# jinseokbae/neural_marionette

Measured on AMD Instinct MI355X. Metric: voxel-frames/sec (64^3, T=16), higher is better.
Workload: dtype f32 (conv products as 3x f16-split MFMA with f32 accumulate, fp32-equivalent; everything else f32); 1 GPU; AIST++-shaped synthetic clips 64^3 T=16 B=4/GPU, full NeuralMarionette.forward (detector + 11 losses + HSVRNNBVH.encode, best-of-10), fp32, random-init weights; grid=64, T=16, clips_per_gpu=4, global_clips=4, conv_mode=split16, parallelism=clip-sharded x1 (no data-path collective)

## Files before the change

### neural_marionette_amd/csrc/nm_conv.hip

```cpp
#include "nm_common.h"
#include "nm_up2c.h"
#include <type_traits>
#include <utility>
#include <vector>

namespace {

#define NM_SPLIT_SCALE 2048.0f

struct ConvParams {
    const float* in; const float* in_scale; const float* in_shift; float in_slope;
    int N, ID, IH, IW, Cin;
    const float* w; const float* bias;
    float* out; float* part;
    int OD, OH, OW, Cout, Co_pad;
    int ks, stride, pad;
    int bz_l2, by_l2, bx_l2;
    int nbz, nby, nbx;
    int KC;
    int cin_real;
    int up2;
    int HZ, HY, HX, HV, HVp;
    int CVp;
    int ZP;
    const void* w16;
    int ksplit;
    int st_z, st_y, st_x;
    unsigned st_sx, st_sy, st_pf;
    unsigned st_m_sx, st_m_sy, st_m_pf;
    const float* in_alt; const unsigned char* in_map;
    const float* in2; const float* in2_scale; const float* in2_shift; float in2_slope;
    int in_h, out_h;
#ifdef NM_DIAG
    unsigned long long* stamps;
#endif
};

__device__ __forceinline__ void lds_barrier() { asm volatile("s_waitcnt lgkmcnt(0)\n\ts_barrier" ::: "memory"); }

__device__ __forceinline__ float lrelu(float v, float slope) { return v > 0.f ? v : v * slope; }


template <bool IH = false>
__device__ __forceinline__ f32x4 load_raw(const ConvParams& p, int n, int z, int y, int x, int c) {
    return nm_ld4<IH>(p.in, ((((size_t)n * p.ID + z) * p.IH + y) * p.IW + x) * p.Cin + c);
}

__device__ __forceinline__ f32x4 apply_act(const ConvParams& p, f32x4 v, const f32x4& sc, const f32x4& sh) {
    if (p.in_scale) {
#pragma unroll
        for (int j = 0; j < 4; ++j) v[j] = __builtin_fmaf(v[j], sc[j], sh[j]);
    }
    if (p.in_slope != 1.0f) {
#pragma unroll
        for (int j = 0; j < 4; ++j) v[j] = fmaxf(v[j], v[j] * p.in_slope);
    }
    return v;
}

__device__ __forceinline__ f32x4 sum_act2(const ConvParams& p, f32x4 a, const f32x4& sca, const f32x4& sha, f32x4 b, const f32x4& scb, const f32x4& shb) {
#pragma unroll
    for (int j = 0; j < 4; ++j) {
        float u = a[j], v = b[j];
        if (p.in_scale) { u = u * sca[j]; u = u + sha[j]; }
        if (p.in_slope != 1.0f) u = u > 0.f ? u : u * p.in_slope;
        if (p.in2_scale) { v = v * scb[j]; v = v + shb[j]; }
        if (p.in2_slope != 1.0f) v = v > 0.f ? v : v * p.in2_slope;
        a[j] = u + v;
    }
    return a;
}

template <bool IH = false>
__device__ __forceinline__ f32x4 load_act(const ConvParams& p, int n, int z, int y, int x, int c) {
    f32x4 v = nm_ld4<IH>(p.in, ((((size_t)n * p.ID + z) * p.IH + y) * p.IW + x) * p.Cin + c);
    f32x4 sc = {0.f, 0.f, 0.f, 0.f}, sh = sc;
    if (p.in_scale) {
        sc = *reinterpret_cast<const f32x4*>(p.in_scale + (size_t)n * p.Cin + c);
        sh = *reinterpret_cast<const f32x4*>(p.in_shift + (size_t)n * p.Cin + c);
    }
    return apply_act(p, v, sc, sh);
}

// ... 2105 lines not shown
            NM_MFMA2(accl[0][0], bh0[i], al0[i]);  if constexpr (bnext) bh0[j] = lds_read16_untracked<BN>(vb);
            NM_MFMA2(accl[0][1], bh1[i], al0[i]);  if constexpr (bnext) bh1[j] = lds_read16_untracked<BN + 32 * 16>(vb);
            NM_MFMA2(acc[1][0], bh0[i], ah1[i]);  if constexpr (bnext) bl0[j] = lds_read16_untracked<BN + 128 * 16>(vb);
            NM_MFMA2(acc[1][1], bh1[i], ah1[i]);  if constexpr (bnext) bl1[j] = lds_read16_untracked<BN + 160 * 16>(vb);
            NM_MFMA2(accl[1][0], bl0[i], ah1[i]);
            NM_MFMA2(accl[1][1], bl1[i], ah1[i]);
            NM_MFMA2(accl[1][0], bh0[i], al1[i]);
            NM_MFMA2(accl[1][1], bh1[i], al1[i]);
            if constexpr (t == 8) {
                NM_PSTAMP(1 + 2 * g);
                asm volatile("s_barrier" ::: "memory");
                __builtin_amdgcn_sched_barrier(0);
                NM_PSTAMP(2 + 2 * g);
            }
        });
        gpar ^= 1;
        if (has_next) {
            ah0[0] = lds_read16_untracked<0>(van); al0[0] = lds_read16_untracked<LO>(van);
            ah1[0] = lds_read16_untracked<YO>(van); al1[0] = lds_read16_untracked<LO + YO>(van);
        }
        if (cur.cb == C16 - 1) {
            const Work& w = cur.w;
            NM_PSTAMP(8);
#pragma unroll
            for (int nt = 0; nt < 2; ++nt) {
                float s1[16], s2[16];
#pragma unroll
                for (int mt = 0; mt < 2; ++mt) {
                    const size_t dst = ((((size_t)w.n * p.OD + w.oz0 + vz) * p.OH + w.oy0 + 2 * wave + mt) * p.OW + w.ox0 + vx) * (size_t)p.Cout +
                                       w.cg * 64 + nt * 32 + 4 * h;
#pragma unroll
                    for (int k4 = 0; k4 < 4; ++k4) {
                        const f32x4 b4 = *reinterpret_cast<const f32x4*>(lbias + w.cg * 64 + nt * 32 + 8 * k4 + 4 * h);
                        f32x4 v;
#pragma unroll
                        for (int e = 0; e < 4; e += 2) {
                            const f32x2 a2 = f32x2{acc[mt][nt][4 * k4 + e], acc[mt][nt][4 * k4 + e + 1]};
                            const f32x2 l2 = f32x2{accl[mt][nt][4 * k4 + e], accl[mt][nt][4 * k4 + e + 1]};
                            const f32x2 v2 = (a2 + l2 * (1.0f / NM_SPLIT_SCALE)) + f32x2{b4[e], b4[e + 1]};
                            const f32x2 q2 = v2 * v2;
                            v[e] = v2[0]; v[e + 1] = v2[1];
                            if (mt == 0) { s1[4 * k4 + e] = v2[0]; s1[4 * k4 + e + 1] = v2[1]; s2[4 * k4 + e] = q2[0]; s2[4 * k4 + e + 1] = q2[1]; }
                            else {
                                const f32x2 t1 = f32x2{s1[4 * k4 + e], s1[4 * k4 + e + 1]} + v2, t2 = f32x2{s2[4 * k4 + e], s2[4 * k4 + e + 1]} + q2;
                                s1[4 * k4 + e] = t1[0]; s1[4 * k4 + e + 1] = t1[1]; s2[4 * k4 + e] = t2[0]; s2[4 * k4 + e + 1] = t2[1];
                            }
                            acc[mt][nt][4 * k4 + e] = 0.f; acc[mt][nt][4 * k4 + e + 1] = 0.f; accl[mt][nt][4 * k4 + e] = 0.f; accl[mt][nt][4 * k4 + e + 1] = 0.f;
                        }
                        *reinterpret_cast<f32x4*>(p.out + dst + 8 * k4) = v;
                    }
                }
                if (nt == 0) NM_PSTAMP(9); else NM_PSTAMP(11);
                if (p.part) {
                    dpp_sum32_many(s1); dpp_sum32_many(s2);
                    if (l31 == 16) {
#pragma unroll
                        for (int r = 0; r < 16; ++r)
                            *reinterpret_cast<f32x2*>(red + (wave * 64 + nt * 32 + (r & 3) + 8 * (r >> 2) + 4 * h) * 2) = f32x2{s1[r], s2[r]};
                    }
                }
                if (nt == 0) NM_PSTAMP(10);
            }
            NM_PSTAMP(12);
            lds_barrier();
            NM_PSTAMP(13);
            if (p.part && tid < 64) {
                float a = 0.f, b = 0.f;
#pragma unroll
                for (int q = 0; q < 4; ++q) { a += red[(q * 64 + tid) * 2]; b += red[(q * 64 + tid) * 2 + 1]; }
                const int br = ((w.oz0 >> 2) * nby + (w.oy0 >> 3)) * nbx + (w.ox0 >> 3);
                float* dp = p.part + (((size_t)w.n * nbr + br) * p.Cout + w.cg * 64 + tid) * 2;
                dp[0] = a; dp[1] = b;
            }
        }
        NM_PSTAMP(7);
#ifdef NM_DIAG
        ++step_no;
#endif
        if (!has_next) break;
        cur = nxt; hb ^= 1;
    }
}

template <int IO = 0>
__global__ __launch_bounds__(512, 1) void conv_f16q2_kernel(ConvParams p) {
    constexpr bool IH = (IO & 1) != 0, OH = (IO & 2) != 0;
    constexpr unsigned EB = IH ? 2u : 4u;
    constexpr int HV = 600, ZP = 100, HX = 10;
    constexpr int WB = 27 * 2 * 64;
    constexpr int NP = IH ? 5 : 10;
    constexpr int NCH = IH ? 8 : 4;
    constexpr int NWL = 14;
    constexpr int NA = IH ? 4 : 2;
    extern __shared__ f32x4 lds[];
    half8* ldh = reinterpret_cast<half8*>(lds);
    half8* ldb = ldh + 4 * HV;
    float* red = reinterpret_cast<float*>(ldb + 2 * WB);
    float* lbias = red + 512;
    const int tid = threadIdx.x, lane = tid & 63, wave = __builtin_amdgcn_readfirstlane(tid >> 6);
    const int h = lane >> 5, l31 = lane & 31;
    const int C16 = p.Cin >> 4;
    const int ncg = p.Cout >> 6;
    const int nbx = p.OW >> 3, nby = p.OH >> 3, nbz = p.OD >> 2, nbr = nbx * nby * nbz;
    const int total = p.N * nbr * ncg;
    const int per = (total + (int)gridDim.x - 1) / (int)gridDim.x;
    const int id_first = (int)blockIdx.x * per, id_last = min(total, id_first + per);
    if (id_first >= id_last) return;

    struct Work { int n, oz0, oy0, ox0, cg; };
    const bool tiled = p.st_x != 0;
    auto decode = [&](int id) {
        Work w;
        if (tiled) {
            const BrickPos bp = super_tile_item(p, (int)blockIdx.x, id - id_first, per, nbz, nby, nbx);
            w.cg = 0; w.n = bp.n; w.ox0 = bp.bx << 3; w.oy0 = bp.by << 3; w.oz0 = bp.bz << 2;
            return w;
        }
        w.cg = id % ncg; const int bid = id / ncg;
        w.n = bid / nbr; const int br = bid % nbr;
        w.ox0 = (br % nbx) << 3; w.oy0 = ((br / nbx) % nby) << 3; w.oz0 = (br / (nbx * nby)) << 2;
        return w;
    };
    auto next_work = [&](Work w, int id) {
        if (tiled) return decode(id);
        if (++w.cg == ncg) {
            w.cg = 0;
            if ((w.ox0 += 8) == p.OW) { w.ox0 = 0; if ((w.oy0 += 8) == p.OH) { w.oy0 = 0; if ((w.oz0 += 4) == p.OD) { w.oz0 = 0; ++w.n; } } }
        }
        return w;
    };
    struct Step { Work w; int id, cb; };
    auto advance = [&](Step& st) {
        if (st.cb + 1 < C16) { ++st.cb; return true; }
        if (st.id + 1 >= id_last) return false;
        st.cb = 0; ++st.id; st.w = next_work(st.w, st.id);
        return true;
    };

    if (wave >= 4) {
        const int pt = tid - 256, pw = wave - 4;
        const half8* __restrict__ w8 = reinterpret_cast<const half8*>(p.w);
        const size_t plane = (size_t)p.Co_pad;
        const int sub = IH ? (pt & 1) : (pt & 3);
        int pc_slot[NP], pc_rel[NP], pc_pos[NP];
#pragma unroll
        for (int k = 0; k < NP; ++k) {
            const int v = IH ? (pt >> 1) + 128 * k : (pt >> 2) + 64 * k, vc = min(v, HV - 1);
            const int hz = vc / 100, r = vc % 100, hy = r / 10, hx = r % 10;
            pc_slot[k] = (IH ? sub : (sub >> 1)) * HV + hz * ZP + hy * HX + hx;
            pc_rel[k] = ((hz * p.IH + hy) * p.IW + hx) * p.Cin + NCH * sub;
            pc_pos[k] = (v < HV) ? (hz | (hy << 8) | (hx << 16)) : -1;
        }
        f32x4 raw[2][NP], sc[2][NA / 2], sh[2][NA / 2], wreg[NWL];
#pragma unroll
        for (int i = 0; i < NWL; ++i) wreg[i] = f32x4{0.f, 0.f, 0.f, 0.f};
        const bool has_affine = p.in_scale != nullptr;
        const unsigned rel111 = (unsigned)(((p.IH + 1) * p.IW + 1) * p.Cin) * EB;
        auto inside_mask = [&](const Work& w) {
            unsigned m = 0;
#pragma unroll
            for (int k = 0; k < NP; ++k) {
                const int hz = pc_pos[k] & 0xff, hy = (pc_pos[k] >> 8) & 0xff, hx = pc_pos[k] >> 16;
                const bool in = pc_pos[k] >= 0 && (unsigned)(w.oz0 - 1 + hz) < (unsigned)p.ID && (unsigned)(w.oy0 - 1 + hy) < (unsigned)p.IH &&
                                (unsigned)(w.ox0 - 1 + hx) < (unsigned)p.IW;
                m |= (in ? 1u : 0u) << k;
            }
// ... 588 lines not shown
    return e;
}

double conv_flops(const ConvParams& p, double taps) { return 2.0 * p.N * (double)p.OD * p.OH * p.OW * p.Cout * (double)p.cin_real * taps; }

template <int MT, int NT>
int launch_t(const ConvParams& p, const Tiling& t, dim3 grid, hipStream_t s) {
    static NmDeviceOnce attr_set;
    if (int rc = nm_raise_lds_limit(attr_set, 160 * 1024, "hipFuncSetAttribute(conv)", &conv_mfma_kernel<MT, NT>)) return rc;
    NmProfScope prof(s, conv_flops(p, (double)p.ks * p.ks * p.ks), (MT - 1) * 2 + (NT - 1));
    hipLaunchKernelGGL((conv_mfma_kernel<MT, NT>), grid, dim3(256), t.lds_bytes, s, p);
    return nm_check_hip(hipGetLastError(), "conv_mfma launch");
}

void choose_super_tile(ConvParams& p, int nblocks, int nbz, int nby, int nbx) {
    p.st_z = p.st_y = p.st_x = 0;
    p.st_sx = p.st_sy = p.st_pf = p.st_m_sx = p.st_m_sy = p.st_m_pf = 0;
    if (nblocks % 8) return;
    const int gs = nblocks / 8;
    const int sz = gs == 64 ? 4 : gs == 32 ? 2 : 0;
    if (!sz || nbz % sz || nby % 4 || nbx % 4) return;
    const long long st = (long long)p.N * (nbz / sz) * (nby / 4) * (nbx / 4);
    if (st % 8 || st / 8 * nblocks != (long long)p.N * nbz * nby * nbx) return;
    p.st_z = sz; p.st_y = 4; p.st_x = 4;
    const unsigned SX = (unsigned)nbx / 4u, SY = (unsigned)nby / 4u, pf = SX * SY * (unsigned)(nbz / sz);
    const unsigned long long smax = 8ull * (unsigned long long)(((long long)p.N * nbz * nby * nbx + nblocks - 1) / nblocks) + 8ull;
    auto magic = [](unsigned d) { return d == 1u ? 0u : (unsigned)((0x100000000ull + d - 1ull) / d); };
    if (smax * pf < 0x100000000ull) {
        p.st_sx = SX; p.st_sy = SY; p.st_pf = pf; p.st_m_sx = magic(SX); p.st_m_sy = magic(SY); p.st_m_pf = magic(pf);
    }
}


template <int MT, int NT, int KS, bool UP2, bool SINGLE, int IO = 0>
int launch_f16s_impl(const ConvParams& p_in, const Tiling& t, dim3 grid, hipStream_t s) {
    ConvParams p = p_in;
    static NmDeviceOnce attr_set;
    if (int rc = nm_raise_lds_limit(attr_set, 160 * 1024, "hipFuncSetAttribute(conv_f16s)", &conv_f16s_kernel<MT, NT, KS, UP2, SINGLE, IO>)) return rc;
    dim3 pgrid(min(grid.x, 512u), grid.y);
    choose_super_tile(p, (int)pgrid.x, p.nbz, p.nby, p.nbx);
    NmProfScope prof(s, conv_flops(p, (double)p.ks * p.ks * p.ks), UP2 ? 10 + (NT - 1) : 5 + (NT - 1));
    hipLaunchKernelGGL((conv_f16s_kernel<MT, NT, KS, UP2, SINGLE, IO>), pgrid, dim3(256), t.lds_bytes, s, p);
    return nm_check_hip(hipGetLastError(), "conv_f16s launch");
}
int io16_unsupported(const char* k, const ConvParams& p) {
    nm_set_error("%s: no instantiation for bfloat16 input=%d / output=%d in this conv mode / layer shape (16-bit storage needs conv mode 4)", k, p.in_h, p.out_h);
    return NM_ERR_UNSUPPORTED;
}
template <int MT, int NT, int KS, bool UP2>
int launch_f16s(const ConvParams& p, const Tiling& t, dim3 grid, hipStream_t s) {
    const int io = (p.in_h ? 1 : 0) | (p.out_h ? 2 : 0);
    if (io) {
        if (!nm_ls().single) return io16_unsupported("conv_f16s", p);
        if constexpr (KS == 1 && !UP2) { if (io == 3) return launch_f16s_impl<MT, NT, KS, UP2, true, 3>(p, t, grid, s); }
        if constexpr (KS == 3 && UP2 && NT == 2) { if (io == 2) return launch_f16s_impl<MT, NT, KS, UP2, true, 2>(p, t, grid, s); }
        return io16_unsupported("conv_f16s", p);
    }
    return nm_ls().single ? launch_f16s_impl<MT, NT, KS, UP2, true>(p, t, grid, s) : launch_f16s_impl<MT, NT, KS, UP2, false>(p, t, grid, s);
}

template <int NT, bool SINGLE>
int launch_pool_f16s_impl(const ConvParams& p, dim3 grid, hipStream_t s) {
    const int io = (p.in_h ? 1 : 0) | (p.out_h ? 2 : 0);
    if (io && (!SINGLE || p.Cin > 128 || p.in2 || p.in_map || !(io & 1))) return io16_unsupported("conv_pool_f16q", p);
    NmProfScope prof(s, conv_flops(p, 8.0), 8);
    if (io) {
        if constexpr (SINGLE) {
            if (io == 3) hipLaunchKernelGGL((conv_pool_f16q_kernel<NT, true, false, 3>), grid, dim3(256), 0, s, p);
            else hipLaunchKernelGGL((conv_pool_f16q_kernel<NT, true, false, 1>), grid, dim3(256), 0, s, p);
        }
    } else
    if (nm_ls().pool_q && p.Cin <= 128) {
        if (p.in2) hipLaunchKernelGGL((conv_pool_f16q_kernel<NT, SINGLE, true>), grid, dim3(256), 0, s, p);
        else hipLaunchKernelGGL((conv_pool_f16q_kernel<NT, SINGLE, false>), grid, dim3(256), 0, s, p);
    } else
    hipLaunchKernelGGL((conv_pool_f16s_kernel<NT, SINGLE>), grid, dim3(256), 0, s, p);
    return nm_check_hip(hipGetLastError(), "conv_pool_f16s launch");
}
template <int NT>
int launch_pool_f16s(const ConvParams& p, dim3 grid, hipStream_t s) {
    return nm_ls().single ? launch_pool_f16s_impl<NT, true>(p, grid, s) : launch_pool_f16s_impl<NT, false>(p, grid, s);
}

template <auto KERNEL>
int launch_persistent(const char* what_attr, const char* what_launch, int variant, bool super_tile, const ConvParams& p_in,
                      size_t lds_bytes, int work_items, hipStream_t s, int wgs_cap) {
    static NmDeviceOnce attr_set;
    if (int rc = nm_raise_lds_limit(attr_set, 160 * 1024, what_attr, KERNEL)) return rc;
    const int cus = nm_num_cus();
    if (!cus) return NM_ERR_HIP;
    ConvParams p = p_in;
    const int wgs = wgs_cap > 0 && wgs_cap < cus ? min(cus, max(8, wgs_cap & ~7)) : cus;
    dim3 grid((unsigned)min(work_items, wgs));
    if (super_tile) choose_super_tile(p, (int)grid.x, p.OD / 4, p.OH / 8, p.OW / 8);
    NmProfScope prof(s, conv_flops(p, 27.0), variant);
    hipLaunchKernelGGL(KERNEL, grid, dim3(512), lds_bytes, s, p);
    return nm_check_hip(hipGetLastError(), what_launch);
}

template <bool SINGLE, int IO = 0>
int launch_f16p_impl(const ConvParams& p, int work_items, hipStream_t s, int wgs_cap) {
    const size_t lds_bytes = (size_t)8 * 600 * 16 + (size_t)3 * 9 * 4 * 32 * 16 + (size_t)(256 + p.Cout) * sizeof(float);
    return launch_persistent<&conv_f16p_kernel<SINGLE, IO>>("hipFuncSetAttribute(conv_f16p)", "conv_f16p launch", 7, p.Cout == 32, p, lds_bytes, work_items, s, wgs_cap);
}
int launch_f16p(const ConvParams& p, int work_items, hipStream_t s, int wgs_cap) {
    const int io = (p.in_h ? 1 : 0) | (p.out_h ? 2 : 0);
    if (io) {
        if (io != 3 || !nm_ls().single) return io16_unsupported("conv_f16p", p);
        return launch_f16p_impl<true, 3>(p, work_items, s, wgs_cap);
    }
    return nm_ls().single ? launch_f16p_impl<true>(p, work_items, s, wgs_cap) : launch_f16p_impl<false>(p, work_items, s, wgs_cap);
}

int launch_f16p2_impl(const ConvParams& p, int work_items, hipStream_t s, int wgs_cap) {
    const size_t lds_bytes = (size_t)8 * 600 * 16 + (size_t)2 * 9 * 4 * 64 * 16 + (size_t)(512 + p.Cout) * sizeof(float);
    return launch_persistent<&conv_f16p2_kernel>("hipFuncSetAttribute(conv_f16p2)", "conv_f16p2 launch", 9, p.Cout == 64, p, lds_bytes, work_items, s, wgs_cap);
}
template <int IO>
int launch_f16q2_impl(const ConvParams& p, int work_items, hipStream_t s, int wgs_cap) {
    const size_t lds_bytes = (size_t)4 * 600 * 16 + (size_t)2 * 27 * 2 * 64 * 16 + (size_t)(512 + p.Cout) * sizeof(float);
    if (lds_bytes > 160 * 1024) { nm_set_error("conv_f16q2: %d output channels exceed the LDS budget", p.Cout); return NM_ERR_UNSUPPORTED; }
    return launch_persistent<&conv_f16q2_kernel<IO>>("hipFuncSetAttribute(conv_f16q2)", "conv_f16q2 launch", 14, p.Cout == 64, p, lds_bytes, work_items, s, wgs_cap);
}
template <int IO, int C16T>
int launch_f16r_impl(const ConvParams& p, int work_items, hipStream_t s, int wgs_cap) {
    const size_t lds_bytes = (size_t)4 * 600 * 16 + (size_t)27 * C16T * 64 * 16 + (size_t)(512 + 32) * sizeof(float) + 2048 + 256 + 1024;
    return launch_persistent<&conv_f16r_kernel<IO, C16T>>("hipFuncSetAttribute(conv_f16r)", "conv_f16r launch", 15, true, p, lds_bytes, work_items, s, wgs_cap);
}
int launch_f16p2(const ConvParams& p, int work_items, hipStream_t s, int wgs_cap) {
    const int io = (p.in_h ? 1 : 0) | (p.out_h ? 2 : 0);
    if (io && (io != 3 || !nm_ls().single)) return io16_unsupported("conv_f16p2", p);
    if (nm_ls().single) return io ? launch_f16q2_impl<3>(p, work_items, s, wgs_cap) : launch_f16q2_impl<0>(p, work_items, s, wgs_cap);
    return launch_f16p2_impl(p, work_items, s, wgs_cap);
}

#ifdef NM_DIAG
unsigned long long* g_stamps = nullptr;
#endif

}

#ifdef NM_DIAG
extern "C" void nm_diag_set_stamps(void* p) { g_stamps = static_cast<unsigned long long*>(p); }
#endif
void nm_conv_set_mode(int mode) { NmLaunchState& l = nm_ls(); l.conv_mode = mode ? 1 : 0; l.f16p_all = mode == 2; l.single = mode == 3 || mode == 4; l.store16 = mode == 4; }
int nm_conv_get_mode() { const NmLaunchState& l = nm_ls(); return l.conv_mode && l.single ? (l.store16 ? 4 : 3) : (l.conv_mode && l.f16p_all ? 2 : l.conv_mode); }
int nm_conv_single() { return nm_ls().conv_mode && nm_ls().single; }

int nm_launch_pack_conv_weight16(const float* w, int Cout, int Cin, int ks, void* packed, int Co_pad, hipStream_t s) {
    if (Co_pad % 32 || Cout > Co_pad) { nm_set_error("pack_conv_weight16: bad padding Cout=%d/%d", Cout, Co_pad); return NM_ERR_ARG; }
    size_t total = (size_t)ks * ks * ks * ((Cin + 15) / 16) * 2 * Co_pad * 8;
    int blocks = (int)min((total + 255) / 256, (size_t)2048);
    hipLaunchKernelGGL(pack_conv_weight16_kernel, dim3(blocks), dim3(256), 0, s, w, Cout, Cin, ks, reinterpret_cast<_Float16*>(packed), Co_pad);
    return nm_check_hip(hipGetLastError(), "pack_conv_weight16 launch");
}

__global__ __launch_bounds__(256) void pack_jobs_kernel(const NmPackJob* __restrict__ jobs, int njobs) {
    int lo = 0, hi = njobs - 1;
    while (lo < hi) { const int mid = (lo + hi + 1) >> 1; if (jobs[mid].blk0 <= (int)blockIdx.x) lo = mid; else hi = mid - 1; }
    const NmPackJob j = jobs[lo];
    const int lb = blockIdx.x - j.blk0, taps = j.ks * j.ks * j.ks;
    auto W = [&](int co, int ci, int tap) -> float {
        if (co >= j.Cout || ci >= j.Cin) return 0.f;
        if (j.src_rows > 0 && ((j.flip ? ci : co) >= j.src_rows || (j.flip ? co : ci) >= j.src_cin)) return 0.f;
        return j.flip ? j.src[((size_t)ci * j.src_cin + co) * taps + (taps - 1 - tap)] : j.src[((size_t)co * j.src_cin + ci) * taps + tap];
    };
    const size_t total32 = (size_t)taps * j.Cin_pad * j.Co_pad;
    for (size_t i = (size_t)lb * 256 + threadIdx.x; i < total32; i += (size_t)j.nblk * 256) {
        const int e = i & 3; size_t r = i >> 2;
        const int co = r % j.Co_pad; r /= j.Co_pad;
        const int q = r % (j.Cin_pad / 4), tap = r / (j.Cin_pad / 4);
        j.wp[i] = W(co, q * 4 + e, tap);
    }
    if (j.wp16) {
        _Float16* packed = reinterpret_cast<_Float16*>(j.wp16);
        const int C16 = (j.Cin + 15) >> 4;
        const size_t total16 = (size_t)taps * C16 * 2 * j.Co_pad * 8;
        for (size_t i = (size_t)lb * 256 + threadIdx.x; i < total16; i += (size_t)j.nblk * 256) {
            const int e = i & 7; size_t r = i >> 3;
            const int co = r % j.Co_pad; r /= j.Co_pad;
            const int hh = r & 1; r >>= 1;
            const int cb = r % C16, tap = r / C16;
            const float v = W(co, cb * 16 + hh * 8 + e, tap);
            const _Float16 h = (_Float16)v;
            const _Float16 l = (_Float16)((v - (float)h) * NM_SPLIT_SCALE);
            const size_t base = ((((size_t)tap * C16 + cb) * 4) * j.Co_pad) * 8;
            packed[base + ((size_t)hh * j.Co_pad + co) * 8 + e] = h;
            packed[base + ((size_t)(2 + hh) * j.Co_pad + co) * 8 + e] = l;
        }
    }
}

int nm_pack_job_blocks(const NmPackJob& j) {
    const size_t total = (size_t)j.ks * j.ks * j.ks * j.Cin_pad * j.Co_pad;
// ... 83 lines not shown

void nm_conv_prof_reset() {
    NmLaunchState& l = nm_ls();
    for (const NmProfRec& r : l.prof) { l.event_pool.push_back(r.a); l.event_pool.push_back(r.b); }
    l.prof.clear();
}

int nm_launch_conv(const TensorRef& in, const float* w_packed, const float* bias, float* out,
                   const ConvGeom& g, float* part, hipStream_t s, int cin_real, const void* w_packed16, int out_h, int wgs_cap) {
    if (in.C % 8 != 0 || g.Co_pad % 32 != 0 || g.Cout > g.Co_pad || g.Cout <= 0) {
        nm_set_error("conv: unsupported channels Cin=%d Cout=%d Co_pad=%d", in.C, g.Cout, g.Co_pad);
        return NM_ERR_ARG;
    }
    const int us = g.up2 ? 2 : 1;
    if ((us * in.D + 2 * g.pad - g.ks) / g.stride + 1 != g.OD || (us * in.H + 2 * g.pad - g.ks) / g.stride + 1 != g.OH ||
        (us * in.W + 2 * g.pad - g.ks) / g.stride + 1 != g.OW) {
        nm_set_error("conv: geometry mismatch in=(%d,%d,%d) k=%d s=%d p=%d out=(%d,%d,%d)", in.D, in.H, in.W,
                     g.ks, g.stride, g.pad, g.OD, g.OH, g.OW);
        return NM_ERR_ARG;
    }
    if ((in.scale == nullptr) != (in.shift == nullptr)) { nm_set_error("conv: scale/shift must come together"); return NM_ERR_ARG; }
    if ((in.brickmap || in.p2) && g.up2) { nm_set_error("conv: a brick-sparse input tensor can only feed the k2 s2 split-fp16 pool kernel"); return NM_ERR_ARG; }
    if (use_up2c(g, in.C)) {
        double flops = 2.0 * in.N * (double)g.OD * g.OH * g.OW * g.Cout * (double)(cin_real > 0 ? cin_real : in.C) * 27.0;
        if (nm_up2y_active()) flops *= 0.5;
        NmProfScope prof(s, flops, 12);
        return nm_launch_conv_up2c(in, g.up2c, bias, out, g.Cout, g.Co_pad, part, s, out_h);
    }
    Tiling t = choose_tiling(g, in.C);
    if (t.lds_bytes > 160 * 1024) { nm_set_error("conv: LDS tile %zu B too large", t.lds_bytes); return NM_ERR_UNSUPPORTED; }
    ConvParams p;
    p.in = in.p; p.in_scale = in.scale; p.in_shift = in.shift; p.in_slope = in.slope;
    p.N = in.N; p.ID = in.D; p.IH = in.H; p.IW = in.W; p.Cin = in.C;
    p.w = w_packed; p.bias = bias; p.out = out; p.part = part;
    p.OD = g.OD; p.OH = g.OH; p.OW = g.OW; p.Cout = g.Cout; p.Co_pad = g.Co_pad;
    p.ks = g.ks; p.stride = g.stride; p.pad = g.pad;
    p.bz_l2 = t.bz_l2; p.by_l2 = t.by_l2; p.bx_l2 = t.bx_l2; p.nbz = t.nbz; p.nby = t.nby; p.nbx = t.nbx;
    p.cin_real = cin_real > 0 ? cin_real : in.C;
    p.up2 = g.up2 ? 1 : 0;
    p.st_z = p.st_y = p.st_x = 0;
    p.st_sx = p.st_sy = p.st_pf = p.st_m_sx = p.st_m_sy = p.st_m_pf = 0;
    p.in_alt = in.alt; p.in_map = in.brickmap;
    p.in2 = in.p2; p.in2_scale = in.scale2; p.in2_shift = in.shift2; p.in2_slope = in.slope2;
    p.in_h = in.h; p.out_h = out_h;
    if (in.p2 && !(nm_conv_pool16_eligible(in.C, g.OD, g.OH, g.OW, w_packed16 != nullptr) && g.ks == 2 && g.stride == 2 && g.pad == 0 && !g.up2 && !in.brickmap)) {
        nm_set_error("conv: an un-materialised residual sum can only feed the k2 s2 split-fp16 pool kernel"); return NM_ERR_ARG;
    }
    if (in.brickmap && !(nm_conv_pool16_eligible(in.C, g.OD, g.OH, g.OW, w_packed16 != nullptr) && g.ks == 2 && g.stride == 2 && g.pad == 0 && !g.up2 &&
                         in.alt && in.D % 4 == 0 && in.H % 8 == 0 && in.W % 8 == 0)) {
        nm_set_error("conv: a brick-sparse input tensor can only feed the k2 s2 split-fp16 pool kernel"); return NM_ERR_ARG;
    }
    p.w16 = (nm_ls().conv_mode == 1 && w_packed16 && in.C % 8 == 0 && !g.up2 && t.MT == 1 && (t.KC % 16 == 0 || t.KC == in.C)) ? w_packed16 : nullptr;
    if (p.w16) t.lds_bytes = max(t.lds_bytes, (size_t)(((t.KC + 15) & ~15) / 4) * (t.HVp + t.CVp) * 16);
    p.ksplit = 1;
    if (p.w16) {
        const int top = ((min(g.OD, 1 << t.bz_l2) - 1) << (t.bx_l2 + t.by_l2)) + ((min(g.OH, 1 << t.by_l2) - 1) << t.bx_l2) + min(g.OW, 1 << t.bx_l2) - 1;
        const int rw = top / 32 + 1;
        p.ksplit = rw == 1 ? 4 : (rw == 2 ? 2 : 1);
        if (p.ksplit > 1) t.lds_bytes = max(t.lds_bytes, (size_t)4 * t.NT * 16 * 64 * sizeof(float));
    }
#ifdef NM_DIAG
    p.stamps = g_stamps;
#endif
    p.KC = t.KC; p.HZ = t.HZ; p.HY = t.HY; p.HX = t.HX; p.HV = t.HV; p.HVp = t.HVp; p.CVp = t.CVp; p.ZP = t.HY * t.HX;
    dim3 grid((unsigned)(in.N * t.nbz * t.nby * t.nbx), (unsigned)(g.Co_pad / (t.NT * 32)));
    if (pool16_case(t, in.C, w_packed16 != nullptr) && g.ks == 2 && g.stride == 2 && g.pad == 0 && !g.up2) {
        p.w = static_cast<const float*>(w_packed16);
        return t.NT == 2 ? launch_pool_f16s<2>(p, grid, s) : launch_pool_f16s<1>(p, grid, s);
    }
    const bool k3_bricks = w_packed16 && in.C % 16 == 0 && g.ks == 3 && g.stride == 1 && g.pad == 1 && !g.up2 &&
                           g.OD % 4 == 0 && g.OH % 8 == 0 && g.OW % 8 == 0 && g.OD >= 16;
    if (nm_ls().conv_mode == 1 && k3_bricks && g.Cout % 64 == 0 && !(nm_ls().single && g.Cout > 1024)) {
        const int work = in.N * (g.OD / 4) * (g.OH / 8) * (g.OW / 8) * (g.Cout / 64);
        p.w = static_cast<const float*>(w_packed16);
        return launch_f16p2(p, work, s, wgs_cap);
    }
    if (nm_ls().conv_mode == 1 && nm_ls().single && nm_ls().f16r && k3_bricks &&(in.C == 32 || in.C == 64) && g.Cout == 32 &&
        (p.in_h != 0) == (p.out_h != 0)) {
        const int work = in.N * (g.OD / 4) * (g.OH / 8) * (g.OW / 8);
        p.w = static_cast<const float*>(w_packed16);
        if (in.C == 32) return p.in_h ? launch_f16r_impl<3, 2>(p, work, s, wgs_cap) : launch_f16r_impl<0, 2>(p, work, s, wgs_cap);
        return p.in_h ? launch_f16r_impl<3, 4>(p, work, s, wgs_cap) : launch_f16r_impl<0, 4>(p, work, s, wgs_cap);
    }
    if (nm_ls().conv_mode == 1 && k3_bricks && g.Cout % 32 == 0 && (nm_ls().f16p_all || g.Cout == 32)) {
        const int work = in.N * (g.OD / 4) * (g.OH / 8) * (g.OW / 8) * (g.Cout / 32);
        p.w = static_cast<const float*>(w_packed16);
        return launch_f16p(p, work, s, wgs_cap);
    }
    if (nm_ls().conv_mode == 1 && w_packed16 && in.C % 16 == 0 && t.MT == 2 && t.bx_l2 == 3 && t.by_l2 == 3 && t.bz_l2 == 2 &&
        g.stride == 1 && (g.ks == 1 || g.ks == 3) && t.HZ == g.ks + 3 && t.HY * t.HX * 2 <= 256) {
        Tiling t16 = t;
        const int area = t.HY * t.HX;
        p.ZP = area + ((4 - (area & 15)) & 15);
        const int hv = t.HZ * p.ZP;
        p.HVp = hv + ((2 - (hv & 7)) & 7);
        const bool blds = (t.NT == 1 && g.ks == 3);
        const size_t bbytes = blds ? (size_t)2 * 9 * 4 * 32 * 16 : 0;
        t16.lds_bytes = max(blds ? (size_t)4 * p.HVp * 16 + bbytes : (size_t)4 * (p.HVp + t.CVp) * 16, (size_t)4 * 64 * 2 * sizeof(float));
        if (t16.lds_bytes <= 80 * 1024) {
            p.w = static_cast<const float*>(w_packed16);
            if (g.ks == 3 && g.up2) return t.NT == 2 ? launch_f16s<2, 2, 3, true>(p, t16, grid, s) : launch_f16s<2, 1, 3, true>(p, t16, grid, s);
            if (g.ks == 3) return t.NT == 2 ? launch_f16s<2, 2, 3, false>(p, t16, grid, s) : launch_f16s<2, 1, 3, false>(p, t16, grid, s);
            if (!g.up2) return t.NT == 2 ? launch_f16s<2, 2, 1, false>(p, t16, grid, s) : launch_f16s<2, 1, 1, false>(p, t16, grid, s);
        }
        p.HVp = t.HVp;
    }
    if (p.in_h || p.out_h) return io16_unsupported("conv (fp32 MFMA kernel)", p);
    if (t.MT == 2 && t.NT == 2) return launch_t<2, 2>(p, t, grid, s);
    if (t.MT == 2 && t.NT == 1) return launch_t<2, 1>(p, t, grid, s);
    if (t.MT == 1 && t.NT == 2) return launch_t<1, 2>(p, t, grid, s);
    return launch_t<1, 1>(p, t, grid, s);
}

int nm_occ_blocks_per_frame(int G) { return (G / 8) * (G / 8) * (G / 4); }

int nm_launch_pack_occ_weight(const float* w_oidhw, int Cout, float* tmp, float* packed, int Co_pad, hipStream_t s) {
    hipLaunchKernelGGL(extract_occ_weight_kernel, dim3((Cout * 125 + 255) / 256), dim3(256), 0, s, w_oidhw, Cout, tmp);
    int rc = nm_check_hip(hipGetLastError(), "extract_occ_weight launch");
    if (rc) return rc;
    rc = nm_launch_pack_conv_weight(tmp, Cout, 125, 1, packed, 128, Co_pad, s);
    if (rc) return rc;
    hipLaunchKernelGGL(pack_occ_weight16_kernel, dim3(64), dim3(256), 0, s, tmp, Cout, Co_pad, reinterpret_cast<_Float16*>(packed + (size_t)128 * Co_pad));
    return nm_check_hip(hipGetLastError(), "pack_occ_weight16 launch");
}

int nm_launch_conv_k5occ(const float* occ, int N, int G, const float* w_packed, const float* field, float* out, int Cout,
                         int Co_pad, float* part, hipStream_t s, unsigned char* brickmap, const float* field_part, unsigned char* flags, int out_h) {
    if (G % 8 || Co_pad % 32 || Cout > Co_pad) { nm_set_error("conv_k5occ: unsupported G=%d Cout=%d", G, Cout); return NM_ERR_ARG; }
    OccParams p; p.occ = occ; p.w = w_packed; p.field = field; p.out = out; p.part = part; p.N = N; p.G = G; p.Cout = Cout; p.Co_pad = Co_pad;
    p.brickmap = brickmap; p.field_part = field_part; p.flags = nullptr; p.row_walk = 0;
    if (brickmap && flags && G <= 128 && G % 8 == 0 && nm_ls().occ_flags) {
        hipLaunchKernelGGL(occ_brick_flags_kernel, dim3((unsigned)(N * (G >> 2))), dim3(256), 0, s, occ, G, flags);
        p.flags = flags; p.row_walk = nm_ls().occ_flags >= 2 ? 1 : 0;
    }
    if (brickmap && (nm_ls().conv_mode != 1 || (part && !field_part))) {
        nm_set_error("conv_k5occ: the brick-sparse output exists on the split-fp16 kernel only and needs the field's partial sums"); return NM_ERR_ARG;
    }
    const int NT = (Co_pad % 64 == 0) ? 2 : 1;
    dim3 grid((unsigned)(N * nm_occ_blocks_per_frame(G)), (unsigned)(Co_pad / (NT * 32)));
    if (p.row_walk) grid.x /= (unsigned)(G >> 3);
    if (out_h && (!(nm_ls().conv_mode == 1 && nm_ls().single) || brickmap || Cout % 4)) {
        nm_set_error("conv_k5occ: bfloat16 output needs conv mode 4, the dense (training) form and Cout %% 4 == 0"); return NM_ERR_UNSUPPORTED;
    }
    NmProfScope prof(s, 2.0 * N * (double)G * G * G * Cout * 4.0 * 125.0, 4);
    if (out_h) {
        if (NT == 2) hipLaunchKernelGGL((conv_k5occ_f16_kernel<2, true, false, true>), grid, dim3(256), 0, s, p);
        else hipLaunchKernelGGL((conv_k5occ_f16_kernel<1, true, false, true>), grid, dim3(256), 0, s, p);
    } else
    if (nm_ls().conv_mode == 1 && p.row_walk) {
        if (NT == 2) { if (nm_ls().single) hipLaunchKernelGGL((conv_k5occ_f16_kernel<2, true, true>), grid, dim3(256), 0, s, p); else hipLaunchKernelGGL((conv_k5occ_f16_kernel<2, false, true>), grid, dim3(256), 0, s, p); }
        else { if (nm_ls().single) hipLaunchKernelGGL((conv_k5occ_f16_kernel<1, true, true>), grid, dim3(256), 0, s, p); else hipLaunchKernelGGL((conv_k5occ_f16_kernel<1, false, true>), grid, dim3(256), 0, s, p); }
    } else if (nm_ls().conv_mode == 1) {
        if (NT == 2) { if (nm_ls().single) hipLaunchKernelGGL((conv_k5occ_f16_kernel<2, true>), grid, dim3(256), 0, s, p); else hipLaunchKernelGGL((conv_k5occ_f16_kernel<2>), grid, dim3(256), 0, s, p); }
        else { if (nm_ls().single) hipLaunchKernelGGL((conv_k5occ_f16_kernel<1, true>), grid, dim3(256), 0, s, p); else hipLaunchKernelGGL((conv_k5occ_f16_kernel<1>), grid, dim3(256), 0, s, p); }
    } else if (NT == 2) hipLaunchKernelGGL((conv_k5occ_kernel<2>), grid, dim3(256), 0, s, p);
    else hipLaunchKernelGGL((conv_k5occ_kernel<1>), grid, dim3(256), 0, s, p);
    return nm_check_hip(hipGetLastError(), "conv_k5occ launch");
}
```

Before: 4154 voxel-frames/s.

## Add 8-deep z-brick persistent conv kernel for Cout=32 3x3x3 layers

```diff
diff --git a/neural_marionette_amd/csrc/nm_conv.hip b/neural_marionette_amd/csrc/nm_conv.hip
--- a/neural_marionette_amd/csrc/nm_conv.hip
+++ b/neural_marionette_amd/csrc/nm_conv.hip
@@ -1,4 +1,5 @@
 #include "nm_common.h"
+#include "nm_f16p8_plan.h"
 #include "nm_up2c.h"
 #include <type_traits>
 #include <utility>
@@ -2270,6 +2271,332 @@
     }
 }
 
+__global__ __launch_bounds__(512, 1) void conv_f16p8_kernel(ConvParams p) {
+    namespace pl = nm_f16p8;
+    constexpr int HV = pl::kHaloVoxels, ZP = 100, HX = 10;
+    constexpr int GB = pl::kWeightBufSlots;
+    constexpr int NP = pl::kPieces;
+    static_assert(HV == 10 * ZP && ZP == 10 * HX, "10 x 10 x 10 halo tile");
+    static_assert(NP * 256 >= 4 * HV && (NP - 1) * 256 < 4 * HV, "pieces cover the tile");
+    extern __shared__ f32x4 lds[];
+    half8* ldh = reinterpret_cast<half8*>(lds);
+    half8* ldb = ldh + pl::kHaloSlots;
+    float* red = reinterpret_cast<float*>(ldb + pl::kWeightSlots);
+    float* lbias = red + pl::kRedFloats;
+    const int tid = threadIdx.x, lane = tid & 63, wave = __builtin_amdgcn_readfirstlane(tid >> 6);
+    const int h = lane >> 5, l31 = lane & 31;
+    const int C16 = p.Cin >> 4;
+    const int nbx = p.OW >> 3, nby = p.OH >> 3, nbz = p.OD >> 3, nbr = nbx * nby * nbz;
+    const int total = p.N * nbr;
+    const int per = (total + (int)gridDim.x - 1) / (int)gridDim.x;
+    const int id_first = (int)blockIdx.x * per, id_last = min(total, id_first + per);
+    if (id_first >= id_last) return;
+    const int items = id_last - id_first;
+
+    struct Work { int n, oz0, oy0, ox0; };
+    const bool tiled = p.st_x != 0;
+    auto decode = [&](int id) {
+        Work w;
+        if (tiled) {
+            const BrickPos bp = super_tile_item(p, (int)blockIdx.x, id - id_first, per, nbz, nby, nbx);
+            w.n = bp.n; w.ox0 = bp.bx << 3; w.oy0 = bp.by << 3; w.oz0 = bp.bz << 3;
+            return w;
+        }
+        w.n = id / nbr; const int br = id % nbr;
+        w.ox0 = (br % nbx) << 3; w.oy0 = ((br / nbx) % nby) << 3; w.oz0 = (br / (nbx * nby)) << 3;
+        return w;
+    };
+    auto next_work = [&](Work w, int id) {
+        if (tiled) return decode(id);
+        if ((w.ox0 += 8) == p.OW) { w.ox0 = 0; if ((w.oy0 += 8) == p.OH) { w.oy0 = 0; if ((w.oz0 += 8) == p.OD) { w.oz0 = 0; ++w.n; } } }
+        return w;
+    };
+    struct Step { Work w; pl::Cursor c; };
+    auto advance = [&](Step& st) {
+        const int item = st.c.item;
+        if (!pl::next_step(st.c, items, C16)) return false;
+        if (st.c.item != item) st.w = next_work(st.w, id_first + st.c.item);
+        return true;
+    };
+
+    if (wave >= 4) {
+        const int pt = tid - 256, pw = wave - 4;
+        const half8* __restrict__ w8 = reinterpret_cast<const half8*>(p.w);
+        const size_t plane = (size_t)p.Co_pad;
+        const int lane_off = h * (int)plane + l31;
+        const int quad = pt & 3;
+        int pc_slot[NP], pc_rel[NP], pc_pos[NP];
+#pragma unroll
+        for (int k = 0; k < NP; ++k) {
+            const int v = (pt >> 2) + 64 * k, vc = min(v, HV - 1);
+            const int hz = vc / 100, r = vc % 100, hy = r / 10, hx = r % 10;
+            pc_slot[k] = (quad >> 1) * HV + hz * ZP + hy * HX + hx;
+            pc_rel[k] = ((hz * p.IH + hy) * p.IW + hx) * p.Cin + 4 * quad;
+            pc_pos[k] = (v < HV) ? (hz | (hy << 8) | (hx << 16)) : -1;
+        }
+        f32x4 raw[NP], sc, sh, wreg[4];
+#pragma unroll
+        for (int i = 0; i < 4; ++i) wreg[i] = f32x4{0.f, 0.f, 0.f, 0.f};
+        const bool has_affine = p.in_scale != nullptr;
+        const unsigned rel111 = (unsigned)(((p.IH + 1) * p.IW + 1) * p.Cin) * 4u;
+        auto inside_mask = [&](const Work& w) {
+            unsigned m = 0;
+#pragma unroll
+            for (int k = 0; k < NP; ++k) {
+                const int hz = pc_pos[k] & 0xff, hy = (pc_pos[k] >> 8) & 0xff, hx = pc_pos[k] >> 16;
+                const bool in = pc_pos[k] >= 0 && (unsigned)(w.oz0 - 1 + hz) < (unsigned)p.ID && (unsigned)(w.oy0 - 1 + hy) < (unsigned)p.IH &&
+                                (unsigned)(w.ox0 - 1 + hx) < (unsigned)p.IW;
+                m |= (in ? 1u : 0u) << k;
+            }
+            return m;
+        };
+        auto tile_base = [&](const Work& w, int cb) {
+            return p.in + (size_t)(((((long long)w.n * p.ID + (w.oz0 - 1)) * p.IH + (w.oy0 - 1)) * p.IW + (w.ox0 - 1)) * (long long)p.Cin + cb * 16);
+        };
+        auto load_piece = [&](const float* base, unsigned mask, auto K) {
+            constexpr int k = decltype(K)::value;
+            raw[k] = load16_untracked(base, ((mask >> k) & 1) ? (unsigned)pc_rel[k] * 4u : rel111);
+        };
+        auto load_affine = [&](const Work& w, int cb) {
+            const float* ps = has_affine ? p.in_scale + (size_t)w.n * p.Cin + cb * 16 : p.in;
+            const float* ph = has_affine ? p.in_shift + (size_t)w.n * p.Cin + cb * 16 : p.in;
+            sc = load16_untracked(ps, 16u * quad);
+            sh = load16_untracked(ph, 16u * quad);
+        };
+#define NM_PRODUCER8_WAIT(N) asm volatile("s_waitcnt vmcnt(" #N ")" \
+            : "+v"(raw[0]), "+v"(raw[1]), "+v"(raw[2]), "+v"(raw[3]), "+v"(raw[4]), "+v"(raw[5]), "+v"(raw[6]), "+v"(raw[7]), \
+              "+v"(raw[8]), "+v"(raw[9]), "+v"(raw[10]), "+v"(raw[11]), "+v"(raw[12]), "+v"(raw[13]), "+v"(raw[14]), "+v"(raw[15]), \
+              "+v"(sc), "+v"(sh), "+v"(wreg[0]), "+v"(wreg[1]), "+v"(wreg[2]), "+v"(wreg[3]) :: "memory")
+        auto convert = [&](int buf, unsigned mask, auto K) {
+            constexpr int k = decltype(K)::value;
+            half4v hi4, lo4;
+            const float keep = ((mask >> k) & 1) ? 1.f : 0.f;
+#pragma unroll
+            for (int e = 0; e < 4; e += 2) {
+                float v0 = raw[k][e], v1 = raw[k][e + 1];
+                if (has_affine) { v0 = __builtin_fmaf(v0, sc[e], sh[e]); v1 = __builtin_fmaf(v1, sc[e + 1], sh[e + 1]); }
+                v0 = fmaxf(v0 * keep, (v0 * keep) * p.in_slope); v1 = fmaxf(v1 * keep, (v1 * keep) * p.in_slope);
+                half2v hv = __builtin_convertvector(f32x2{v0, v1}, half2v);
+                asm volatile("" : "+v"(hv));
+                const float t0 = v0 * NM_SPLIT_SCALE, t1 = v1 * NM_SPLIT_SCALE;
+                hi4[e] = hv[0]; hi4[e + 1] = hv[1];
+                lo4[e] = (_Float16)__builtin_fmaf((float)hv[0], -NM_SPLIT_SCALE, t0);
+                lo4[e + 1] = (_Float16)__builtin_fmaf((float)hv[1], -NM_SPLIT_SCALE, t1);
+            }
+            if (pc_pos[k] >= 0) {
+                half4v* dst = reinterpret_cast<half4v*>(ldh + buf * 4 * HV + pc_slot[k]) + (quad & 1);
+                dst[0] = hi4;
+                dst[4 * HV] = lo4;
+            }
+        };
+        constexpr int NW = 4;
+        unsigned w_src[NW], w_dst[NW], w_src6, w_dst6;
+        {
+            auto piece = [&](int j, unsigned& src, unsigned& dst) {
+                const int t = j >> 1, lo = j & 1;
+                src = (unsigned)(((size_t)t * C16 * 4 + lo * 2) * plane + lane_off) * 16u;
+                dst = (unsigned)(t * 128 + lo * 64 + lane) * 16u;
+            };
+#pragma unroll
+            for (int i = 0; i < NW; ++i) piece(min(pw + 4 * i, 2 * pl::group_taps(0) - 1), w_src[i], w_dst[i]);
+            piece(min(pw + 4 * (NW - 1), 2 * pl::group_taps(pl::kGroups - 1) - 1), w_src6, w_dst6);
+        }
+        static_assert(4 * NW >= 2 * pl::kGroupTaps && 4 * (NW - 1) <= 2 * pl::group_taps(pl::kGroups - 1), "only the last slot of a wave can pass a group's end");
+        auto load_b_group = [&](int cb, auto G) {
+            constexpr int g = decltype(G)::value;
+            constexpr bool short_group = pl::group_taps(g) < pl::kGroupTaps;
+            const char* base = reinterpret_cast<const char*>(w8 + ((size_t)pl::group_first(g) * C16 * 4 + (size_t)cb * 4) * plane);
+            const float* src[NW];
+#pragma unroll
+            for (int i = 0; i < NW; ++i) src[i] = reinterpret_cast<const float*>(base + ((short_group && i == NW - 1) ? w_src6 : w_src[i]));
+            __builtin_amdgcn_sched_barrier(0);
+#pragma unroll
+            for (int i = 0; i < NW; ++i) wreg[i] = load16_untracked(src[i]);
+            __builtin_amdgcn_sched_barrier(0);
+        };
+        auto store_b_group = [&](auto G) {
+            constexpr int g = decltype(G)::value;
+            constexpr bool short_group = pl::group_taps(g) < pl::kGroupTaps;
+            __builtin_amdgcn_sched_barrier(0);
+            char* lbase = reinterpret_cast<char*>(ldb + (g & 1) * GB);
+#pragma unroll
+            for (int i = 0; i < NW; ++i) *reinterpret_cast<f32x4*>(lbase + ((short_group && i == NW - 1) ? w_dst6 : w_dst[i])) = wreg[i];
+        };
+
+        Step cur; cur.w = decode(id_first); cur.c.item = 0; cur.c.cb = 0;
+        int hb = 0;
+        Step s1 = cur; bool has1 = advance(s1);
+        Step s2 = s1;  bool has2 = has1 && advance(s2);
+        unsigned m_cvt = inside_mask(cur.w), m_ld = m_cvt;
+        for (int c = pt; c < 32; c += 256) lbias[c] = p.bias ? p.bias[c] : 0.f;
+        load_b_group(0, ic<0>{});
+        load_affine(cur.w, 0);
+        { const float* b = tile_base(cur.w, 0); static_for<NP>([&](auto K) { load_piece(b, m_cvt, K); }); }
+        NM_PRODUCER8_WAIT(0);
+        store_b_group(ic<0>{});
+        static_for<NP>([&](auto K) { convert(0, m_cvt, K); });
+        m_cvt = inside_mask(s1.w);
+        load_affine(s1.w, s1.c.cb);
+        { const float* b = tile_base(s1.w, s1.c.cb); static_for<NP>([&](auto K) { load_piece(b, m_cvt, K); }); }
+        lds_barrier();
+        for (;;) {
+            if (s2.w.n != s1.w.n || s2.w.oz0 != s1.w.oz0 || s2.w.oy0 != s1.w.oy0 || s2.w.ox0 != s1.w.ox0) m_ld = inside_mask(s2.w);
+            else m_ld = m_cvt;
+            const float* b2 = tile_base(s2.w, s2.c.cb);
+            static_for<pl::kGroups>([&](auto G) {
+                constexpr int g = decltype(G)::value, gn = (g + 1) % pl::kGroups;
+                constexpr int k0 = pl::piece_first(g), nk = pl::piece_first(g + 1) - k0;
+                constexpr bool last = g == pl::kGroups - 1;
+                if constexpr (last) load_b_group(s1.c.cb, ic<gn>{}); else load_b_group(cur.c.cb, ic<gn>{});
+                if constexpr (g == 0) { NM_PRODUCER8_WAIT(4); }
+                static_for<nk>([&](auto K) { convert(hb ^ 1, m_cvt, ic<decltype(K)::value + k0>{}); load_piece(b2, m_ld, ic<decltype(K)::value + k0>{}); });
+                if constexpr (last) load_affine(s2.w, s2.c.cb);
+                static_assert((nk == 4 && !last) || (nk == 5 && !last) || (nk == 2 && last), "the counted waits below are written for this deal");
+                if constexpr (nk == 5) { NM_PRODUCER8_WAIT(5); } else { NM_PRODUCER8_WAIT(4); }
+                store_b_group(ic<gn>{});
+                lds_barrier();
+            });
+            if (pl::brick_end(cur.c.cb, C16)) lds_barrier();
+            if (!has1) break;
+            cur = s1; s1 = s2; has1 = has2; has2 = has2 && advance(s2);
+            m_cvt = m_ld; hb ^= 1;
+        }
+        NM_PRODUCER8_WAIT(0);
+        return;
+    }
+
+    __builtin_amdgcn_s_setprio(3);
+    int arow0;
+    {
+        const int c = l31 >> 2;
+        const int x = (((0x96 >> c) & 1) << 2) + (l31 & 3), z = c >> 1;
+        arow0 = z * ZP + (2 * wave) * HX + x;
+    }
+    const int vx = ((((0x96 >> (l31 >> 2)) & 1) << 2) + (l31 & 3)), vz = l31 >> 3;
+    f32x16 acc[4], accl[4];
+#pragma unroll
+    for (int m = 0; m < 4; ++m)
+#pragma unroll
+        for (int r = 0; r < 16; ++r) { acc[m][r] = 0.f; accl[m][r] = 0.f; }
+
+    Step cur; cur.w = decode(id_first); cur.c.item = 0; cur.c.cb = 0;
+    int hb = 0;
+    lds_barrier();
+
+    constexpr int LO = 2 * HV * 16;
+    constexpr int YO = HX * 16;
+    constexpr int ZO = 4 * ZP * 16;
+    const unsigned vb = (unsigned)(size_t)(ldb + h * 32 + l31);
+    half8 ah0[2], ah1[2], ah2[2], ah3[2], al0[2], al1[2], al2[2], al3[2], bh[2], bl[2];
+    {
+        const unsigned va = (unsigned)(size_t)(ldh + h * HV + arow0);
+        ah0[0] = lds_read16_untracked<0>(va); ah1[0] = lds_read16_untracked<YO>(va);
+        ah2[0] = lds_read16_untracked<ZO>(va); ah3[0] = lds_read16_untracked<ZO + YO>(va);
+        al0[0] = lds_read16_untracked<LO>(va); al1[0] = lds_read16_untracked<LO + YO>(va);
+        al2[0] = lds_read16_untracked<LO + ZO>(va); al3[0] = lds_read16_untracked<LO + ZO + YO>(va);
+    }
+    const int nbr4 = nbx * nby * (p.OD >> 2);
+    for (;;) {
+        Step nxt = cur;
+        const bool has_next = advance(nxt);
+        const unsigned va = (unsigned)(size_t)(ldh + hb * 4 * HV + h * HV + arow0);
+        const unsigned van = (unsigned)(size_t)(ldh + (hb ^ 1) * 4 * HV + h * HV + arow0);
+        static_for<pl::kTaps>([&](auto TT) {
+            constexpr int tt = decltype(TT)::value, g = pl::group_of(tt), t = pl::tap_in_group(tt), i = tt & 1, j = i ^ 1;
+            constexpr int BT = ((g & 1) * GB + t * 128) * 16;
+            if constexpr (t == 0) {
+                bh[i] = lds_read16_untracked<BT>(vb); bl[i] = lds_read16_untracked<BT + 64 * 16>(vb);
+            }
+            asm volatile("s_waitcnt lgkmcnt(0)"
+                         : "+v"(ah0[i]), "+v"(ah1[i]), "+v"(ah2[i]), "+v"(ah3[i]), "+v"(al0[i]), "+v"(al1[i]), "+v"(al2[i]), "+v"(al3[i]),
+                           "+v"(bh[i]), "+v"(bl[i]) :: "memory");
+            __builtin_amdgcn_sched_barrier(0);
+            constexpr int u = tt + 1, uz = (u < pl::kTaps) ? u / 9 : 0, ut = (u < pl::kTaps) ? u % 9 : 0;
+            constexpr int AO = (uz * ZP + (ut / 3) * HX + (ut % 3)) * 16;
+            constexpr bool anext = u < pl::kTaps;
+            constexpr bool bnext = !pl::group_end(tt);
+            constexpr int BN = BT + 128 * 16;
+            NM_MFMA2(acc[0], bh[i], ah0[i]);   if constexpr (bnext) bh[j] = lds_read16_untracked<BN>(vb);
+                                               if constexpr (anext) ah0[j] = lds_read16_untracked<AO>(va);
+            NM_MFMA2(acc[1], bh[i], ah1[i]);   if constexpr (bnext) bl[j] = lds_read16_untracked<BN + 64 * 16>(vb);
+                                               if constexpr (anext) ah1[j] = lds_read16_untracked<AO + YO>(va);
+            NM_MFMA2(acc[2], bh[i], ah2[i]);   if constexpr (anext) ah2[j] = lds_read16_untracked<AO + ZO>(va);
+            NM_MFMA2(acc[3], bh[i], ah3[i]);   if constexpr (anext) ah3[j] = lds_read16_untracked<AO + ZO + YO>(va);
+            NM_MFMA2(accl[0], bl[i], ah0[i]);  if constexpr (anext) al0[j] = lds_read16_untracked<AO + LO>(va);
+            NM_MFMA2(accl[1], bl[i], ah1[i]);  if constexpr (anext) al1[j] = lds_read16_untracked<AO + LO + YO>(va);
+            NM_MFMA2(accl[2], bl[i], ah2[i]);  if constexpr (anext) al2[j] = lds_read16_untracked<AO + LO + ZO>(va);
+            NM_MFMA2(accl[3], bl[i], ah3[i]);  if constexpr (anext) al3[j] = lds_read16_untracked<AO + LO + ZO + YO>(va);
+            NM_MFMA2(accl[0], bh[i], al0[i]);
+            NM_MFMA2(accl[1], bh[i], al1[i]);
+            NM_MFMA2(accl[2], bh[i], al2[i]);
+            NM_MFMA2(accl[3], bh[i], al3[i]);
+            if constexpr (pl::group_end(tt)) {
+                asm volatile("s_barrier" ::: "memory");
+                __builtin_amdgcn_sched_barrier(0);
+            }
+        });
+        static_assert(((pl::kTaps - 1) & 1) == 0, "tap 26 computes from slot 0, tap 0 of the next step reads into it");
+        if (has_next) {
+            ah0[0] = lds_read16_untracked<0>(van); ah1[0] = lds_read16_untracked<YO>(van);
+            ah2[0] = lds_read16_untracked<ZO>(van); ah3[0] = lds_read16_untracked<ZO + YO>(van);
+            al0[0] = lds_read16_untracked<LO>(van); al1[0] = lds_read16_untracked<LO + YO>(van);
+            al2[0] = lds_read16_untracked<LO + ZO>(van); al3[0] = lds_read16_untracked<LO + ZO + YO>(van);
+        }
+        if (pl::brick_end(cur.c.cb, C16)) {
+            const Work& w = cur.w;
+#pragma unroll
+            for (int zh = 0; zh < 2; ++zh) {
+                float s1[16], s2[16];
+#pragma unroll
+                for (int my = 0; my < 2; ++my) {
+                    const int m = 2 * zh + my;
+                    const size_t dst = ((((size_t)w.n * p.OD + w.oz0 + 4 * zh + vz) * p.OH + w.oy0 + 2 * wave + my) * p.OW + w.ox0 + vx) * (size_t)32 + 4 * h;
+#pragma unroll
+                    for (int k4 = 0; k4 < 4; ++k4) {
+                        const f32x4 b4 = *reinterpret_cast<const f32x4*>(lbias + 8 * k4 + 4 * h);
+                        f32x4 v;
+#pragma unroll
+                        for (int e = 0; e < 4; e += 2) {
+                            const f32x2 a2 = f32x2{acc[m][4 * k4 + e], acc[m][4 * k4 + e + 1]};
+                            const f32x2 l2 = f32x2{accl[m][4 * k4 + e], accl[m][4 * k4 + e + 1]};
+                            const f32x2 v2 = (a2 + l2 * (1.0f / NM_SPLIT_SCALE)) + f32x2{b4[e], b4[e + 1]};
+                            const f32x2 q2 = v2 * v2;
+                            v[e] = v2[0]; v[e + 1] = v2[1];
+                            if (my == 0) { s1[4 * k4 + e] = v2[0]; s1[4 * k4 + e + 1] = v2[1]; s2[4 * k4 + e] = q2[0]; s2[4 * k4 + e + 1] = q2[1]; }
+                            else {
+                                const f32x2 t1 = f32x2{s1[4 * k4 + e], s1[4 * k4 + e + 1]} + v2, t2 = f32x2{s2[4 * k4 + e], s2[4 * k4 + e + 1]} + q2;
+                                s1[4 * k4 + e] = t1[0]; s1[4 * k4 + e + 1] = t1[1]; s2[4 * k4 + e] = t2[0]; s2[4 * k4 + e + 1] = t2[1];
+                            }
+                            acc[m][4 * k4 + e] = 0.f; acc[m][4 * k4 + e + 1] = 0.f; accl[m][4 * k4 + e] = 0.f; accl[m][4 * k4 + e + 1] = 0.f;
+                        }
+                        *reinterpret_cast<f32x4*>(p.out + dst + 8 * k4) = v;
+                    }
+                }
+                if (p.part) {
+                    dpp_sum32_many(s1); dpp_sum32_many(s2);
+                    if (l31 == 16) {
+#pragma unroll
+                        for (int r = 0; r < 16; ++r)
+                            *reinterpret_cast<f32x2*>(red + ((zh * 4 + wave) * 32 + (r & 3) + 8 * (r >> 2) + 4 * h) * 2) = f32x2{s1[r], s2[r]};
+                    }
+                }
+            }
+            lds_barrier();
+            if (p.part && tid < 64) {
+                const int zh = tid >> 5, c = tid & 31;
+                float a = 0.f, b = 0.f;
+#pragma unroll
+                for (int q = 0; q < 4; ++q) { a += red[((zh * 4 + q) * 32 + c) * 2]; b += red[((zh * 4 + q) * 32 + c) * 2 + 1]; }
+                const int br = (((w.oz0 >> 2) + zh) * nby + (w.oy0 >> 3)) * nbx + (w.ox0 >> 3);
+                float* dp = p.part + (((size_t)w.n * nbr4 + br) * 32 + c) * 2;
+                dp[0] = a; dp[1] = b;
+            }
+        }
+        if (!has_next) break;
+        cur = nxt; hb ^= 1;
+    }
+}
+
 template <int IO = 0>
 __global__ __launch_bounds__(512, 1) void conv_f16q2_kernel(ConvParams p) {
     constexpr bool IH = (IO & 1) != 0, OH = (IO & 2) != 0;
@@ -3024,7 +3351,7 @@
     return nm_ls().single ? launch_pool_f16s_impl<NT, true>(p, grid, s) : launch_pool_f16s_impl<NT, false>(p, grid, s);
 }
 
-template <auto KERNEL>
+template <auto KERNEL, int BRICK_Z = 4>
 int launch_persistent(const char* what_attr, const char* what_launch, int variant, bool super_tile, const ConvParams& p_in,
                       size_t lds_bytes, int work_items, hipStream_t s, int wgs_cap) {
     static NmDeviceOnce attr_set;
@@ -3034,7 +3361,7 @@
     ConvParams p = p_in;
     const int wgs = wgs_cap > 0 && wgs_cap < cus ? min(cus, max(8, wgs_cap & ~7)) : cus;
     dim3 grid((unsigned)min(work_items, wgs));
-    if (super_tile) choose_super_tile(p, (int)grid.x, p.OD / 4, p.OH / 8, p.OW / 8);
+    if (super_tile) choose_super_tile(p, (int)grid.x, p.OD / BRICK_Z, p.OH / 8, p.OW / 8);
     NmProfScope prof(s, conv_flops(p, 27.0), variant);
     hipLaunchKernelGGL(KERNEL, grid, dim3(512), lds_bytes, s, p);
     return nm_check_hip(hipGetLastError(), what_launch);
@@ -3052,6 +3379,10 @@
         return launch_f16p_impl<true, 3>(p, work_items, s, wgs_cap);
     }
     return nm_ls().single ? launch_f16p_impl<true>(p, work_items, s, wgs_cap) : launch_f16p_impl<false>(p, work_items, s, wgs_cap);
+}
+
+int launch_f16p8(const ConvParams& p, int work_items, hipStream_t s, int wgs_cap) {
+    return launch_persistent<&conv_f16p8_kernel, 8>("hipFuncSetAttribute(conv_f16p8)", "conv_f16p8 launch", 7, true, p, (size_t)nm_f16p8::kLdsBytes, work_items, s, wgs_cap);
 }
 
 int launch_f16p2_impl(const ConvParams& p, int work_items, hipStream_t s, int wgs_cap) {
@@ -3301,6 +3632,11 @@
         if (in.C == 32) return p.in_h ? launch_f16r_impl<3, 2>(p, work, s, wgs_cap) : launch_f16r_impl<0, 2>(p, work, s, wgs_cap);
         return p.in_h ? launch_f16r_impl<3, 4>(p, work, s, wgs_cap) : launch_f16r_impl<0, 4>(p, work, s, wgs_cap);
     }
+    if (nm_ls().conv_mode == 1 && !nm_ls().single && k3_bricks && g.Cout == 32 && g.OD % 8 == 0 && !p.in_h && !p.out_h) {
+        const int work = in.N * (g.OD / 8) * (g.OH / 8) * (g.OW / 8);
+        p.w = static_cast<const float*>(w_packed16);
+        return launch_f16p8(p, work, s, wgs_cap);
+    }
     if (nm_ls().conv_mode == 1 && k3_bricks && g.Cout % 32 == 0 && (nm_ls().f16p_all || g.Cout == 32)) {
         const int work = in.N * (g.OD / 4) * (g.OH / 8) * (g.OW / 8) * (g.Cout / 32);
         p.w = static_cast<const float*>(w_packed16);
diff --git a/neural_marionette_amd/csrc/nm_f16p8_plan.h b/neural_marionette_amd/csrc/nm_f16p8_plan.h
--- /dev/null
+++ b/neural_marionette_amd/csrc/nm_f16p8_plan.h
@@ -0,0 +1,46 @@
+#pragma once
+
+#ifdef __HIPCC__
+#define NM_PLAN_FN __host__ __device__ constexpr
+#else
+#define NM_PLAN_FN constexpr
+#endif
+
+namespace nm_f16p8 {
+
+constexpr int kTaps = 27;
+constexpr int kGroupTaps = 7;
+constexpr int kGroups = 4;
+constexpr int kPieces = 16;
+
+constexpr int kHaloVoxels = 1000;
+constexpr int kHaloSlots = 2 * 4 * kHaloVoxels;
+constexpr int kWeightBufSlots = kGroupTaps * 4 * 32;
+constexpr int kWeightSlots = 2 * kWeightBufSlots;
+constexpr int kRedFloats = 2 * 4 * 32 * 2;
+constexpr int kBiasFloats = 32;
+constexpr unsigned long kLdsBytes = (unsigned long)(kHaloSlots + kWeightSlots) * 16 + (unsigned long)(kRedFloats + kBiasFloats) * 4;
+static_assert(kLdsBytes == 158848 && kLdsBytes <= 160 * 1024, "LDS budget of gfx950: 163 840 B per workgroup");
+
+NM_PLAN_FN int group_first(int g) { return g * kGroupTaps < kTaps ? g * kGroupTaps : kTaps; }
+NM_PLAN_FN int group_taps(int g) { return group_first(g + 1) - group_first(g); }
+NM_PLAN_FN int group_of(int tap) { return tap / kGroupTaps; }
+NM_PLAN_FN int tap_in_group(int tap) { return tap % kGroupTaps; }
+NM_PLAN_FN bool group_end(int tap) { return tap + 1 == group_first(group_of(tap) + 1); }
+NM_PLAN_FN int piece_first(int g) { return g == 0 ? 0 : g == 1 ? 4 : g == 2 ? 9 : g == 3 ? 14 : kPieces; }
+NM_PLAN_FN bool brick_end(int cb, int C16) { return cb == C16 - 1; }
+
+static_assert(group_first(kGroups) == kTaps && group_taps(3) == 6 && group_taps(0) == 7, "7 / 7 / 7 / 6");
+static_assert(kGroups % 2 == 0, "group g in buffer g & 1 needs an even number of groups per step");
+static_assert(group_end(6) && group_end(13) && group_end(20) && group_end(26) && !group_end(0) && !group_end(25), "group ends");
+static_assert(piece_first(kGroups) == kPieces, "every piece is dealt to a group");
+
+struct Cursor { int item, cb; };
+NM_PLAN_FN bool next_step(Cursor& c, int items, int C16) {
+    if (c.cb + 1 < C16) { ++c.cb; return true; }
+    if (c.item + 1 >= items) return false;
+    c.cb = 0; ++c.item;
+    return true;
+}
+
+}
```

Result: faster. 4265 voxel-frames/s (median of 6 runs) (+2.7%).
